# LukasHedegaard/continual-skeletons

Hardware: AMD Instinct MI355X
Metric: clips/sec (ST-GCN clip forward, NTU-60 shape; CoST-GCN online step reported under costgcn_online) (higher is better)
Workload: dtype f32

## Files before the change

### continual-skeletons_amd/blocks.py

```python
import math

import numpy as np
import torch
import torch.nn as nn
from torch.nn.modules.batchnorm import _BatchNorm
from torch.nn.modules.conv import _ConvNd

from . import fold, native


def init_weights(module_, bs=1):
    if isinstance(module_, _ConvNd):
        nn.init.constant_(module_.bias, 0)
        if bs == 1:
            nn.init.kaiming_normal_(module_.weight, mode="fan_out")
        else:
            nn.init.normal_(module_.weight, 0, math.sqrt(2.0 / (module_.weight.numel() * bs)))
    elif isinstance(module_, _BatchNorm):
        nn.init.constant_(module_.weight, bs)
        nn.init.constant_(module_.bias, 0)
    elif isinstance(module_, nn.Linear):
        nn.init.normal_(module_.weight, 0, math.sqrt(2.0 / bs))


def zero(x):
    return 0


def unity(x):
    return x


class _Folded(nn.Module):

    def _watched(self):
        return [self]

    def _snapshot(self):
        tensors, modules, seen = [], [(self._modules, tuple(self._modules.items()))], set()
        for root in self._watched():
            for m in root.modules():
                if id(m) in seen:
                    continue
                seen.add(id(m))
                for d in (m._parameters, m._buffers):
                    for name, t in d.items():
                        tensors.append((d, name, t, None if t is None else t.data_ptr(), None if t is None else t._version))
                modules.append((m._modules, tuple(m._modules.items())))
        return tensors, modules

    @staticmethod
    def _stale(snapshot):
        tensors, modules = snapshot
        for d, name, t, ptr, ver in tensors:
            cur = d.get(name)
            if cur is not t or (t is not None and (cur._version != ver or cur.data_ptr() != ptr)):
                return True
        for d, items in modules:
            if len(d) != len(items):
                return True
            for name, child in items:
                if d.get(name) is not child:
                    return True
        return False

    def _fingerprint(self):
        ts = [t for root in self._watched() for t in list(root.parameters()) + list(root.buffers())]
        return tuple((t.data_ptr(), t._version) for t in ts)

    def _packed_ops(self, device):
        cache = self.__dict__.get("_fold_cache")
        device = str(device)
        if cache is None or cache[0] != device or self._stale(cache[2]):
            ops = {k: (v.to(device) if isinstance(v, torch.Tensor) and not k.endswith("_host") else v)
                   for k, v in self._fold().items()}
            self.__dict__["_fold_cache"] = cache = (device, ops, self._snapshot())
        return cache[1]

    def refold(self):
        self.__dict__.pop("_fold_cache", None)

    def _require_eval(self):
        if self.training:
            raise RuntimeError(
                f"{type(self).__name__}: the MI355X path is inference-only (BatchNorm folded with running "
                "statistics); call .eval() first"
            )


PRECISIONS = ("f32", "bf16x3")


def set_precision(module: nn.Module, precision: str = "f32") -> nn.Module:
    if precision not in PRECISIONS:
        raise ValueError(f"precision must be one of {PRECISIONS}, got {precision!r}")
    blocks_ = [m for m in module.modules() if isinstance(m, SpatioTemporalBlock)]
    if not blocks_:
        raise ValueError("no SpatioTemporalBlock below this module: nothing to set")
    for m in blocks_:
        if precision != "f32" and not (m._native_tail and m.tcn.kernel_size == 9):
            raise NotImplementedError("bf16x3 is built for blocks with the native 9 x 1 temporal conv; the model is unchanged")
    for m in module.modules():
        if isinstance(m, SpatioTemporalBlock) or type(m) is GraphConvolution:
            m.precision = precision
            m.refold()
    return module


class SplitScratch:

    def __init__(self):
        self._bufs = {}

    def get(self, device, floats: int) -> torch.Tensor:
        key = (str(device), torch.cuda.current_stream(device).cuda_stream)
        bufs = self._bufs.setdefault(key, [])
        if not bufs or bufs[-1].numel() < floats:
            bufs.append(torch.empty(int(floats), device=device, dtype=torch.float32))
        return bufs[-1]

    def release(self):
        self._bufs.clear()

    def nbytes(self) -> int:
        return 4 * sum(b.numel() for bufs in self._bufs.values() for b in bufs)


def _scratch_of(module) -> SplitScratch:
    sc = module.__dict__.get("_split_scratch")
    if sc is None:
        sc = module.__dict__["_split_scratch"] = SplitScratch()
    return sc


CLIP_SPLIT_MAX_SEQUENCES = 6


def set_clip_latency_mode(module: nn.Module, split_k: int = 4, gcn_split_k: int = None, max_sequences: int = CLIP_SPLIT_MAX_SEQUENCES) -> nn.Module:
    gcn_split_k = split_k if gcn_split_k is None else gcn_split_k
    for v in (split_k, gcn_split_k):
        if not isinstance(v, int) or v < 0 or v > 32:
            raise ValueError("split_k must be an integer in [0, 32]")
    targets = [m for m in module.modules() if isinstance(m, SpatioTemporalBlock) or type(m) is GraphConvolution]
    if not targets:
        raise ValueError("no SpatioTemporalBlock / GraphConvolution below this module: nothing to set")
    if not isinstance(max_sequences, int) or max_sequences < 1:
        raise ValueError("max_sequences must be a positive integer")
    old = {id(sc): sc for sc in (m.__dict__.get("_split_scratch") for m in targets) if sc is not None}
    for sc in old.values():
        sc.release()
    shared = SplitScratch() if max(split_k, gcn_split_k) > 1 else None
    for m in targets:
        m.clip_split_k = split_k if isinstance(m, SpatioTemporalBlock) else gcn_split_k
        m.clip_split_max_seq = int(max_sequences)
        m.__dict__["_split_scratch"] = shared
    return module


def _check_input(x, channels, name):
    native.require_device_f32(x, name)
    if x.dim() != 4 or x.shape[1] != channels:
        raise RuntimeError(f"{name} must be (N, {channels}, T, V), got {tuple(x.shape)}")


class GraphConvolution(_Folded):

    def __init__(self, in_channels, out_channels, A, bn_momentum=0.1, *args, **kwargs):
        super().__init__()
        self.in_channels = in_channels
        self.out_channels = out_channels
        self.graph_attn = nn.Parameter(torch.ones(A.shape, dtype=torch.float32))
        self.A = nn.Parameter(torch.from_numpy(np.asarray(A).astype(np.float32)), requires_grad=False)
        self.num_subset = 3
        self.g_conv = nn.ModuleList(nn.Conv2d(in_channels, out_channels, 1) for _ in range(self.num_subset))
        for conv in self.g_conv:
            init_weights(conv, bs=self.num_subset)
        if in_channels != out_channels:
            self.gcn_residual = nn.Sequential(
                nn.Conv2d(in_channels, out_channels, 1), nn.BatchNorm2d(out_channels, momentum=bn_momentum)
            )
            init_weights(self.gcn_residual[0], bs=1)
            init_weights(self.gcn_residual[1], bs=1)
        else:
            self.gcn_residual = unity
        self.bn = nn.BatchNorm2d(out_channels, momentum=bn_momentum)
        init_weights(self.bn, bs=1e-6)
        self.relu = nn.ReLU()

    precision = "f32"

    def _fold(self):
        return fold.fold_graph_conv(self.state_dict(), split=self.precision == "bf16x3")

    def _split_applies(self, ops):
        cnt = ops["ell_cnt_host"]
        return (self.precision == "bf16x3" and ops["w_split"] is not None and self.out_channels % 128 == 0
                and int(cnt[0]) <= 1 and int(cnt[1]) <= 1 and int(cnt[2]) <= 4)

    def forward(self, x):
        self._require_eval()
        _check_input(x, self.in_channels, "GraphConvolution input")
        ops = self._packed_ops(x.device)
        n, c, t, v = x.shape
        if v != ops["V"]:
            raise RuntimeError(f"input has V={v} joints, adjacency has {ops['V']}")
        y = torch.empty((n, self.out_channels, t, v), device=x.device, dtype=torch.float32)
        if self._split_applies(ops):
            rc = native.lib().csk_gcn_stage_bf16x3(
                native.ptr(x), native.ptr(y), native.ptr(ops["w_split"]), native.ptr(ops["w_res_split"]), native.ptr(ops["bias"]),
                native.ptr(ops["ell_src"]), native.ptr(ops["ell_val"]), native.ptr(ops["ell_cnt_host"]), ops["ell_w"], n, c,
                self.out_channels, t, v, ops["res_mode"], native.stream_of(x))
            native.check(rc, "csk_gcn_stage_bf16x3")
            return y
        ks = self._clip_ksplit() if n <= self.clip_split_max_seq else 1
        if ks > 1:
            self.stage(x, y, n_seg=n, frames=t, x_strides=(c * t * v, t * v), y_strides=(self.out_channels * t * v, t * v),
                       ksplit=ks, partial=_scratch_of(self).get(x.device, ks * n * self.out_channels * t * v))
            return y
        gcn_stage(x, y, ops, n_seg=n, frames=t, x_strides=(c * t * v, t * v), y_strides=(self.out_channels * t * v, t * v))
        return y

    clip_split_k = 0
    clip_split_max_seq = CLIP_SPLIT_MAX_SEQUENCES

    def _clip_ksplit(self) -> int:
        if self.clip_split_k <= 1 or type(self) is not GraphConvolution or self.in_channels < 16:
            return 1
        return max(1, min(self.clip_split_k, -(-self.in_channels // 8)))

    def stage(self, x, y, n_seg, frames, x_strides, y_strides, ksplit=1, partial=None):
        ops = self._packed_ops(x.device)
        if ksplit > 1:
            rc = native.lib().csk_gcn_stage_splitk_f32(
                native.ptr(x), native.ptr(y), native.ptr(ops["w"]), native.ptr(ops["bias"]), native.ptr(ops["ell_src"]),
                native.ptr(ops["ell_val"]), native.ptr(ops["ell_cnt_host"]), ops["ell_w"], n_seg, ops["c_in"], ops["c_out"], frames,
                ops["V"], x_strides[0], x_strides[1], y_strides[0], y_strides[1], ops["res_mode"], ksplit, native.ptr(partial),
                native.stream_of(x))
            native.check(rc, "csk_gcn_stage_splitk_f32")
            return
        gcn_stage(x, y, ops, n_seg=n_seg, frames=frames, x_strides=x_strides, y_strides=y_strides)


def gcn_stage(x, y, ops, n_seg, frames, x_strides, y_strides, adj_seg_stride=0, adj_per_frame=0):
    rc = native.lib().csk_gcn_stage_f32(
        native.ptr(x), native.ptr(y), native.ptr(ops["w"]), native.ptr(ops["bias"]),
        native.ptr(ops["ell_src"]), native.ptr(ops["ell_val"]), native.ptr(ops["ell_cnt_host"]),
        ops["ell_w"], adj_seg_stride, adj_per_frame, n_seg, ops["c_in"], ops["c_out"], frames, ops["V"],
        x_strides[0], x_strides[1], y_strides[0], y_strides[1], ops["res_mode"], native.stream_of(x),
    )
    native.check(rc, "csk_gcn_stage_f32")


class TemporalConvolution(_Folded):

    def __init__(self, in_channels, out_channels, kernel_size=9, stride=1, padding=4):
        super().__init__()
        self.padding = padding
        self.stride = stride
        self.kernel_size = kernel_size
        self.t_conv = nn.Conv2d(in_channels, out_channels, kernel_size=(kernel_size, 1), padding=(padding, 0),
                                stride=(stride, 1))
        self.bn = nn.BatchNorm2d(out_channels)
        init_weights(self.t_conv, bs=1)
        init_weights(self.bn, bs=1)

    def _fold(self):
        f = fold.fold_temporal_conv(self.state_dict())
        f["bias"] = fold.pad_vec(f["bias"])
        return f

    def forward(self, x):
        self._require_eval()
        _check_input(x, self.t_conv.in_channels, "TemporalConvolution input")
        ops = self._packed_ops(x.device)
        return tcn_stage(x, ops["w"], ops["bias"], ops["c_out"], ops["k"], self.stride, self.padding, relu=False)


def tcn_stage(y, w, bias, c_out, k, stride, pad, relu=True, res_mode=0, x_res=None, w_res=None, res_off=0, out=None,
              split=False, ksplit=1, scratch=None):
    n, c, t_in, v = y.shape
    if t_in + 2 * pad < k:
        raise RuntimeError(f"temporal extent {t_in} (+2*{pad}) shorter than kernel {k}")
    t_out = (t_in + 2 * pad - k) // stride + 1
    if out is None:
        out = torch.empty((n, c_out, t_out, v), device=y.device, dtype=torch.float32)
    elif tuple(out.shape) != (n, c_out, t_out, v) or not out.is_contiguous() or out.dtype != torch.float32 or out.device != y.device:
        raise RuntimeError(f"out must be a contiguous float32 {(n, c_out, t_out, v)} tensor on {y.device}")
    c_res, t_res = (x_res.shape[1], x_res.shape[2]) if x_res is not None else (0, 0)
    if ksplit > 1 and not split:
        if scratch is None:
            raise RuntimeError("tcn_stage: ksplit > 1 needs the owning module's SplitScratch")
        part = scratch.get(y.device, ksplit * n * c_out * t_out * v)
        rc = native.lib().csk_tcn_stage_splitk_f32(
            native.ptr(y), native.ptr(w), native.ptr(x_res), native.ptr(w_res), native.ptr(bias), native.ptr(out),
            n, c, c_out, t_in, v, k, stride, pad, res_mode, c_res, t_res, res_off, int(relu), ksplit, native.ptr(part),
            native.stream_of(y))
        native.check(rc, "csk_tcn_stage_splitk_f32")
        return out
    fn = native.lib().csk_tcn_stage_bf16x3 if split else native.lib().csk_tcn_stage_f32
    rc = fn(native.ptr(y), native.ptr(w), native.ptr(x_res), native.ptr(w_res), native.ptr(bias), native.ptr(out),
            n, c, c_out, t_in, v, k, stride, pad, res_mode, c_res, t_res, res_off, int(relu), native.stream_of(y))
    native.check(rc, "csk_tcn_stage_bf16x3" if split else "csk_tcn_stage_f32")
    return out


class SpatioTemporalBlock(_Folded):

    def __init__(self, in_channels, out_channels, A, stride=1, residual=True, temporal_kernel_size=9,
                 temporal_padding=-1, GraphConv=GraphConvolution, TempConv=TemporalConvolution):
        super().__init__()
        equal_padding = int((temporal_kernel_size - 1) / 2)
        if temporal_padding < 0:
            temporal_padding = equal_padding
            self.residual_shrink = None
        else:
            assert temporal_padding <= equal_padding
            self.residual_shrink = equal_padding - temporal_padding
        self.stride = stride
        self.gcn = GraphConv(in_channels, out_channels, A)
        self.tcn = TempConv(out_channels, out_channels, stride=stride, kernel_size=temporal_kernel_size,
                            padding=temporal_padding)
        self.relu = nn.ReLU()
        if not residual:
            self.residual = zero
        elif (in_channels == out_channels) and (stride == 1):
            self.residual = unity
        else:
            self.residual = TempConv(in_channels, out_channels, kernel_size=1, stride=stride, padding=0)
        self._native_tail = isinstance(self.tcn, TemporalConvolution) and (
            self.residual in (zero, unity) or isinstance(self.residual, TemporalConvolution)
        )

    precision = "f32"
    clip_split_k = 0
    clip_split_max_seq = CLIP_SPLIT_MAX_SEQUENCES

    def _watched(self):
        return [m for m in (self.tcn, self.residual) if isinstance(m, nn.Module)]

    def _fold(self):
        sd = self.state_dict()
        return fold.fold_block_tail(sd, "", has_conv_residual=isinstance(self.residual, TemporalConvolution),
                                    split=self.precision == "bf16x3", stride=self.stride)

    def forward(self, x, out=None):
        self._require_eval()
        native.require_device_f32(x, "SpatioTemporalBlock input")
        if self._few_channels_fusable(x):
            return self._forward_few_channels(x, out)
        y = self.gcn(x)
        if not self._native_tail:
            z = self.tcn(y)
            r = self.residual(x[:, :, self.residual_shrink:-self.residual_shrink] if self.residual_shrink else x)
            return self.relu(z + r)
        ops = self._packed_ops(x.device)
        shrink = self.residual_shrink or 0
        if self.residual is zero:
            mode, xr = 0, None
        elif self.residual is unity:
            mode, xr = 1, x
        else:
            mode, xr = 2, x
        if self.precision == "bf16x3":
            return tcn_stage(y, ops["w_split"], ops["bias"], ops["c_out"], ops["k"], self.stride, self.tcn.padding, relu=True,
                             res_mode=mode, x_res=xr, w_res=ops["w_res_split"], res_off=shrink, out=out, split=True)
        ks = max(1, min(self.clip_split_k, -(-ops["c"] // 8))) if (self.clip_split_k > 1 and ops["k"] == 9 and y.shape[0] <= self.clip_split_max_seq) else 1
        return tcn_stage(y, ops["w"], ops["bias"], ops["c_out"], ops["k"], self.stride, self.tcn.padding, relu=True,
                         res_mode=mode, x_res=xr, w_res=ops["w_res"], res_off=shrink, out=out, ksplit=ks,
                         scratch=_scratch_of(self) if ks > 1 else None)


def _few_channels_fusable(self, x) -> bool:
    if not self.fuse_few_channels or type(self.gcn) is not GraphConvolution or not self._native_tail:
        return False
    if self.gcn.in_channels > 4 or self.residual is not zero or self.stride != 1 or self.precision != "f32" or self.residual_shrink:
        return False
    if x.dim() != 4 or x.shape[3] not in (18, 25) or self.gcn.precision != "f32":
        return False
    if self.clip_split_k > 1 and x.shape[0] <= self.clip_split_max_seq:
        return False
    g, t = self.gcn._packed_ops(x.device), self._packed_ops(x.device)
    return (t["k"] == 9 and self.tcn.padding == 4 and g["res_mode"] == 2 and g["c_out"] % 8 == 0 and g["V"] == x.shape[3]
            and max(int(v) for v in g["ell_cnt_host"][:2]) <= 1 and int(g["ell_cnt_host"][2]) <= 4)


def _forward_few_channels(self, x, out=None):
    _check_input(x, self.gcn.in_channels, "SpatioTemporalBlock input")
    g, t = self.gcn._packed_ops(x.device), self._packed_ops(x.device)
    n, c, tt, v = x.shape
    if out is None:
        out = torch.empty((n, t["c_out"], tt, v), device=x.device, dtype=torch.float32)
    rc = native.lib().csk_block_few_channels_f32(
        native.ptr(x.contiguous()), native.ptr(g["w"]), native.ptr(g["bias"]), native.ptr(g["ell_src"]), native.ptr(g["ell_val"]),
        native.ptr(g["ell_cnt_host"]), g["ell_w"], native.ptr(t["w"]), native.ptr(t["bias"]), native.ptr(out), n, c, g["c_out"],
        t["c_out"], tt, v, self.tcn.padding, native.stream_of(x))
    native.check(rc, "csk_block_few_channels_f32")
    return out


SpatioTemporalBlock.fuse_few_channels = False
SpatioTemporalBlock._few_channels_fusable = _few_channels_fusable
SpatioTemporalBlock._forward_few_channels = _forward_few_channels


def tcn_step_launch(*args):
    native.check(native.lib().csk_tcn_step_f32(*args), "csk_tcn_step_f32")
```

### continual-skeletons_amd/fold.py

```python
from typing import Dict, Optional, Tuple

import numpy as np
import torch

KC = 16
MT = 64
BN_EPS = 1e-5


def _ceil_to(a: int, b: int) -> int:
    return (a + b - 1) // b * b


def bn_affine(weight, bias, mean, var, eps=BN_EPS) -> Tuple[torch.Tensor, torch.Tensor]:
    s = weight.double() / torch.sqrt(var.double() + eps)
    return s, bias.double() - mean.double() * s


def pack_conv_weight(weight: torch.Tensor, scale: torch.Tensor) -> torch.Tensor:
    co, ci, k, _ = weight.shape
    w = weight.double()[:, :, :, 0] * scale[:, None, None]
    out = torch.zeros((k, _ceil_to(ci, KC), _ceil_to(co, MT)), dtype=torch.float64)
    out[:, :ci, :co] = w.permute(2, 1, 0)
    return out.float().contiguous()


SPLIT_KS = 16


def split3_bf16(w32: torch.Tensor):
    h = w32.to(torch.bfloat16)
    r1 = w32 - h.float()
    m = r1.to(torch.bfloat16)
    l = (r1 - m.float()).to(torch.bfloat16)
    return h, m, l


def pack_conv_weight_split(weight: torch.Tensor, scale: torch.Tensor, stride: int = 1) -> torch.Tensor:
    if weight.dim() == 4:
        weight = weight[:, :, :, 0]
    co, ci, k = weight.shape
    if k not in (1, 3, 9):
        raise ValueError(f"split weights are built for the 9 x 1 temporal conv, the 1 x 1 residual convs and the 3 graph-conv "
                         f"subsets, got k = {k}")
    w32 = (weight.double() * scale[:, None, None]).float()
    cpad, mpad = _ceil_to(ci, SPLIT_KS), _ceil_to(co, MT)
    taps = [r for rho in range(min(stride, k)) for r in range(rho, k, stride)] if k > 1 else [0]
    slots = _ceil_to(len(taps), 3)
    full = torch.zeros((mpad, cpad, slots), dtype=torch.float32)
    full[:co, :ci, : len(taps)] = w32[:, :, taps]
    pieces = torch.stack([p.view(torch.int16) for p in split3_bf16(full)], 0)
    out = pieces.view(3, mpad, cpad // SPLIT_KS, 2, 8, slots).permute(2, 5, 0, 3, 1, 4)
    return out.contiguous().reshape(-1)


def pad_vec(v: torch.Tensor) -> torch.Tensor:
    out = torch.zeros(_ceil_to(v.numel(), MT), dtype=torch.float64)
    out[: v.numel()] = v
    return out.float().contiguous()


def ell_from_dense(a_eff: torch.Tensor):
    a = a_eff.detach().cpu().double().numpy()
    three, v, _ = a.shape
    nz = a != 0
    per_col = nz.sum(axis=1)
    cnt = per_col.max(axis=1).astype(np.int32)
    ew = max(1, int(cnt.max()))
    src = np.zeros((three, v, ew), dtype=np.int32)
    val = np.zeros((three, v, ew), dtype=np.float32)
    for i in range(three):
        for w in range(v):
            rows = np.nonzero(nz[i, :, w])[0]
            src[i, w, : len(rows)] = rows
            val[i, w, : len(rows)] = a[i, rows, w]
    return torch.from_numpy(src), torch.from_numpy(val), torch.from_numpy(cnt), ew


def fold_graph_conv(sd: Dict[str, torch.Tensor], p: str = "", split: bool = False) -> dict:
    sd = {k: v.detach().cpu() for k, v in sd.items() if k.startswith(p)}
    s, t = bn_affine(sd[p + "bn.weight"], sd[p + "bn.bias"], sd[p + "bn.running_mean"], sd[p + "bn.running_var"])
    co, ci = sd[p + "g_conv.0.weight"].shape[:2]
    conv_res = (p + "gcn_residual.0.weight") in sd
    r = 4 if conv_res else 3
    w = torch.zeros((r, _ceil_to(ci, KC), _ceil_to(co, MT)), dtype=torch.float64)
    bias = t.clone()
    for i in range(3):
        w[i, :ci, :co] = (sd[f"{p}g_conv.{i}.weight"].double()[:, :, 0, 0] * s[:, None]).t()
        bias += s * sd[f"{p}g_conv.{i}.bias"].double()
    if conv_res:
        sr, tr = bn_affine(sd[p + "gcn_residual.1.weight"], sd[p + "gcn_residual.1.bias"],
                           sd[p + "gcn_residual.1.running_mean"], sd[p + "gcn_residual.1.running_var"])
        w[3, :ci, :co] = (sd[p + "gcn_residual.0.weight"].double()[:, :, 0, 0] * sr[:, None]).t()
        bias += sr * sd[p + "gcn_residual.0.bias"].double() + tr
    a_eff = sd[p + "A"].double() * sd[p + "graph_attn"].double()
    src, val, cnt, ew = ell_from_dense(a_eff)
    out = dict(w=w.float().contiguous(), bias=pad_vec(bias), ell_src=src, ell_val=val, ell_cnt_host=cnt,
               ell_w=ew, c_in=ci, c_out=co, res_mode=2 if conv_res else 1, V=a_eff.shape[-1], w_split=None, w_res_split=None)
    if split:
        one = torch.ones(co, dtype=torch.float64)
        w3 = w[:3, :ci, :co].permute(2, 1, 0).contiguous()
        out["w_split"] = pack_conv_weight_split(w3, one)
        if conv_res:
            out["w_res_split"] = pack_conv_weight_split(w[3, :ci, :co].t().contiguous().unsqueeze(-1), one)
    return out


def fold_temporal_conv(sd: Dict[str, torch.Tensor], p: str = "") -> dict:
    s, t = bn_affine(sd[p + "bn.weight"].cpu(), sd[p + "bn.bias"].cpu(), sd[p + "bn.running_mean"].cpu(),
                     sd[p + "bn.running_var"].cpu())
    wt = sd[p + "t_conv.weight"].detach().cpu()
    bias = s * sd[p + "t_conv.bias"].detach().cpu().double() + t
    return dict(w=pack_conv_weight(wt, s), bias=bias, c_in=wt.shape[1], c_out=wt.shape[0], k=wt.shape[2])


def fold_temporal_conv_split(sd: Dict[str, torch.Tensor], p: str = "", stride: int = 1) -> torch.Tensor:
    s, _ = bn_affine(sd[p + "bn.weight"].cpu(), sd[p + "bn.bias"].cpu(), sd[p + "bn.running_mean"].cpu(),
                     sd[p + "bn.running_var"].cpu())
    return pack_conv_weight_split(sd[p + "t_conv.weight"].detach().cpu(), s, stride)


def fold_block_tail(sd: Dict[str, torch.Tensor], p: str = "", has_conv_residual: Optional[bool] = None,
                    split: bool = False, stride: int = 1) -> dict:
    main = fold_temporal_conv(sd, p + "tcn.")
    out = dict(w=main["w"], k=main["k"], c=main["c_in"], c_out=main["c_out"], w_res=None, c_res=0, w_split=None, w_res_split=None)
    bias = main["bias"]
    if has_conv_residual is None:
        has_conv_residual = (p + "residual.t_conv.weight") in sd
    if has_conv_residual:
        res = fold_temporal_conv(sd, p + "residual.")
        out["w_res"], out["c_res"] = res["w"], res["c_in"]
        bias = bias + res["bias"]
    if split:
        out["w_split"] = fold_temporal_conv_split(sd, p + "tcn.", stride)
        if has_conv_residual:
            out["w_res_split"] = fold_temporal_conv_split(sd, p + "residual.")
    out["bias"] = pad_vec(bias)
    return out


def fold_data_bn(sd: Dict[str, torch.Tensor], p: str = "data_bn."):
    s, t = bn_affine(sd[p + "weight"].cpu(), sd[p + "bias"].cpu(), sd[p + "running_mean"].cpu(),
                     sd[p + "running_var"].cpu())
    return s.float().contiguous(), t.float().contiguous()
```

### continual-skeletons_amd/native.py

```python
import ctypes as C
import os

import torch

_HERE = os.path.dirname(os.path.abspath(__file__))
LIB_PATH = os.path.join(_HERE, "libcskel_hip.so")
ABI_VERSION = 15

_p, _i, _l = C.c_void_p, C.c_int, C.c_int64
SIGNATURES = {
    "csk_abi_version": [],
    "csk_stream_overlap_probe": [C.c_void_p, C.c_void_p, C.c_int, C.POINTER(C.c_float)],
    "csk_gcn_stage_f32": [_p, _p, _p, _p, _p, _p, _p, _i, _l, _i, _i, _i, _i, _i, _i, _l, _l, _l, _l, _i, _p],
    "csk_gcn_stage_splitk_f32": [_p, _p, _p, _p, _p, _p, _p, _i, _i, _i, _i, _i, _i, _l, _l, _l, _l, _i, _i, _p, _p],
    "csk_tcn_stage_f32": [_p, _p, _p, _p, _p, _p, _i, _i, _i, _i, _i, _i, _i, _i, _i, _i, _i, _i, _i, _p],
    "csk_block_few_channels_f32": [_p, _p, _p, _p, _p, _p, _i, _p, _p, _p, _i, _i, _i, _i, _i, _i, _i, _p],
    "csk_tcn_stage_splitk_f32": [_p, _p, _p, _p, _p, _p, _i, _i, _i, _i, _i, _i, _i, _i, _i, _i, _i, _i, _i, _i, _p, _p],
    "csk_conv1x1_f32": [_p, _p, _p, _p, _i, _i, _i, _i, _i, _l, _l, _l, _l, _p],
    "csk_tcn_stage_bf16x3": [_p, _p, _p, _p, _p, _p, _i, _i, _i, _i, _i, _i, _i, _i, _i, _i, _i, _i, _i, _p],
    "csk_gcn_stage_bf16x3": [_p, _p, _p, _p, _p, _p, _p, _p, _i, _i, _i, _i, _i, _i, _i, _p],
    "csk_input_norm_f32": [_p, _p, _p, _p, _i, _i, _i, _i, _i, _l, _l, _p],
    "csk_pool_fc_f32": [_p, _p, _p, _p, _p, _i, _i, _i, _i, _i, _p],
    "csk_fc_f32": [_p, _p, _p, _p, _i, _i, _i, _p],
    "csk_pool_scaled_f32": [_p, _p, _i, _i, _i, _i, C.c_float, _p],
    "csk_agcn_attention_f32": [_p, _p, _p, _p, _i, _i, _i, _i, _l, _l, _i, _l, _p],
    "csk_agcn_embed_attention_f32": [_p, _p, _p, _p, _p, _p, _i, _i, _i, _i, _i, _i, _l, _l, _p],
    "csk_tcn_step_f32": [_p, _i, _i, _i, _i, _p, _p, _i, _i, _i, _p, _p, _p, _i, _i, _i, _i, _l, _i, _i, _i, _i, _i, _p, _p],
    "csk_co_stack_step_f32": [_i, _p, _i, _i, _l, _p],
    "csk_co_block_step_f32": [_p, _i, _i, _i, _p, _p, _p, _p, _p, _i, _i, _p, _i, _i, _p, _p, _i, _i, _p, _i, _i, _i, _i, _i, _l, _p],
    "csk_co_spatial_pool_f32": [_p, _p, _i, _i, _i, _l, _p],
    "csk_co_window_mean_f32": [_p, _p, _l, _i, _i, _i, _p],
    "csk_co_head_step_f32": [_p, _p, _p, _p, _p, _p, _i, _i, _i, _l, _i, _i, _i, _i, _i, _p],
    "csk_input_norm_frames_f32": [_p, _p, _i, _p, _p, _i, _i, _i, _i, _l, _p],

    "csk_fuse_rank_f32": [_p, _i, _i, _i, _i, _l, _l, _p, _p, _p, _p],
    "csk_co_plan_create": [_i, _p, _p, _i, _i, _i, _i, _i, _l, _p, _p, _i, _p, _p, _i, _i, _p, _p],
    "csk_co_plan_destroy": [_p],
    "csk_co_plan_update_weights": [_p, _i, _p, _p, _p, _p, _p],
    "csk_co_plan_reset": [_p],
    "csk_co_plan_counters": [_p, C.POINTER(C.c_int64), _i, _i],
    "csk_co_plan_set_fusion": [_p, _i],
    "csk_co_plan_cycle": [_p, _p, _i, _p, _p, _p, _p, _p],
}
RESTYPES = {"csk_co_plan_create": C.c_void_p, "csk_co_plan_destroy": None, "csk_co_plan_reset": None}


class CoLayer(C.Structure):
    _fields_ = [("c_in", C.c_int32), ("c_out", C.c_int32), ("stride", C.c_int32), ("res_kind", C.c_int32),
                ("gcn_res_mode", C.c_int32), ("ell_w", C.c_int32), ("ell_cnt", C.c_int32 * 3), ("tcn_ksplit", C.c_int32),
                ("y_slots", C.c_int32), ("out_slots", C.c_int32), ("partial_emits", C.c_int32), ("agcn_adj_frames", C.c_int32),
                ("gcn_ksplit", C.c_int32), ("gcn_partial_frames", C.c_int32),
                ("gcn_w", C.c_void_p), ("gcn_bias", C.c_void_p), ("ell_src", C.c_void_p), ("ell_val", C.c_void_p),
                ("tcn_w", C.c_void_p), ("tcn_w_res", C.c_void_p), ("tcn_bias", C.c_void_p),
                ("y_ring", C.c_void_p), ("out_ring", C.c_void_p), ("tcn_partial", C.c_void_p),
                ("agcn_inter", C.c_int32), ("agcn_pad_", C.c_int32), ("agcn_w_pairs", C.c_void_p), ("agcn_b_pairs", C.c_void_p),
                ("agcn_a_sum", C.c_void_p), ("agcn_adj", C.c_void_p)]


_lib = None


def lib():
    global _lib
    if _lib is None:
        if not os.path.exists(LIB_PATH):
            raise RuntimeError(
                f"{LIB_PATH} not found: the HIP library is not built. "
                "Run `python -c 'import __graft_entry__ as g; g.build()'` (needs hipcc); there is no CPU fallback."
            )
        handle = C.CDLL(LIB_PATH)
        for name, args in SIGNATURES.items():
            fn = getattr(handle, name)
            fn.argtypes = args
            fn.restype = RESTYPES.get(name, C.c_int)
        handle.csk_last_error.restype = C.c_char_p
        handle.csk_last_error.argtypes = []
        if handle.csk_abi_version() != ABI_VERSION:
            raise RuntimeError("libcskel_hip.so ABI version mismatch; rebuild it")
        _lib = handle
    return _lib


def check(rc: int, what: str):
    if rc == 0:
        return
    if rc < 0:
        raise RuntimeError(f"{what}: {lib().csk_last_error().decode()}")
    raise RuntimeError(f"{what}: HIP launch failed with hipError_t {rc}")


def ptr(t):
    return None if t is None else C.c_void_p(t.data_ptr())


def stream_of(t: torch.Tensor):
    return C.c_void_p(torch.cuda.current_stream(t.device).cuda_stream)


def require_device_f32(t: torch.Tensor, name: str):
    if not isinstance(t, torch.Tensor):
        raise TypeError(f"{name} must be a torch.Tensor")
    if not t.is_cuda:
        raise RuntimeError(
            f"{name} is on {t.device}: this is the MI355X-native path and has no CPU fallback "
            "(move the module and its inputs to a ROCm device)"
        )
    if t.dtype != torch.float32:
        raise RuntimeError(f"{name} must be float32, got {t.dtype}")
    if not t.is_contiguous():
        raise RuntimeError(f"{name} must be contiguous")
```

### include/cskel.h

```cpp
#ifndef CSKEL_H
#define CSKEL_H

#include <stdint.h>

#ifdef __cplusplus
extern "C" {
#endif

#define CSK_ABI_VERSION 15
#define CSK_KC 8
#define CSK_CPAD 16
#define CSK_MT 64

#define CSK_RES_NONE 0
#define CSK_RES_IDENTITY 1
#define CSK_RES_CONV 2

int csk_abi_version(void);
const char *csk_last_error(void);

int csk_stream_overlap_probe(void *stream_a, void *stream_b, int spin_us, float *ratio);

int csk_gcn_stage_f32(const float *x, float *y, const float *w, const float *bias,
                      const int32_t *ell_src, const float *ell_val, const int32_t *ell_cnt,
                      int ell_w, int64_t adj_seg_stride, int adj_per_frame,
                      int n_seg, int c_in, int c_out, int frames, int V,
                      int64_t x_seg_stride, int64_t x_chan_stride,
                      int64_t y_seg_stride, int64_t y_chan_stride,
                      int res_mode, void *stream);

int csk_gcn_stage_splitk_f32(const float *x, float *y, const float *w, const float *bias, const int32_t *ell_src,
                             const float *ell_val, const int32_t *ell_cnt, int ell_w, int n_seg, int c_in, int c_out,
                             int frames, int V, int64_t x_seg_stride, int64_t x_chan_stride, int64_t y_seg_stride,
                             int64_t y_chan_stride, int res_mode, int ksplit, float *partial, void *stream);

int csk_tcn_stage_f32(const float *y, const float *w, const float *x_res, const float *w_res,
                      const float *bias, float *out,
                      int n_seg, int c, int c_out, int t_in, int V, int k, int stride, int pad,
                      int res_mode, int c_res, int t_res, int res_off, int relu, void *stream);

int csk_block_few_channels_f32(const float *x, const float *gcn_w, const float *gcn_bias, const int32_t *ell_src,
                               const float *ell_val, const int32_t *ell_cnt, int ell_w, const float *tcn_w,
                               const float *tcn_bias, float *out, int n_seg, int c_in, int c_mid, int c_out, int t_in,
                               int V, int pad, void *stream);

int csk_tcn_stage_splitk_f32(const float *y, const float *w, const float *x_res, const float *w_res,
                             const float *bias, float *out,
                             int n_seg, int c, int c_out, int t_in, int V, int k, int stride, int pad,
                             int res_mode, int c_res, int t_res, int res_off, int relu, int ksplit, float *partial,
                             void *stream);

int csk_conv1x1_f32(const float *x, float *y, const float *w, const float *bias, int n_seg, int c_in, int c_out,
                    int frames, int V, int64_t x_seg_stride, int64_t x_chan_stride, int64_t y_seg_stride,
                    int64_t y_chan_stride, void *stream);

int csk_tcn_stage_bf16x3(const float *y, const void *w_split, const float *x_res, const void *w_res_split,
                         const float *bias, float *out,
                         int n_seg, int c, int c_out, int t_in, int V, int k, int stride, int pad,
                         int res_mode, int c_res, int t_res, int res_off, int relu, void *stream);

int csk_gcn_stage_bf16x3(const float *x, float *y, const void *w_split, const void *w_res_split, const float *bias,
                         const int32_t *ell_src, const float *ell_val, const int32_t *ell_cnt, int ell_w,
                         int n_seg, int c_in, int c_out, int frames, int V, int res_mode, void *stream);

int csk_input_norm_f32(const float *x, const float *scale, const float *shift, float *h,
                       int N, int C, int T, int V, int M,
                       int64_t h_seg_stride, int64_t h_chan_stride, void *stream);

int csk_pool_fc_f32(const float *h, const float *fc_w, const float *fc_b, float *feat, float *logits,
                    int N, int M, int C, int TV, int classes, void *stream);

int csk_pool_scaled_f32(const float *h, float *feat, int N, int M, int C, int TV, float scale, void *stream);

int csk_fc_f32(const float *feat, const float *fc_w, const float *fc_b, float *logits,
               int N, int C, int classes, void *stream);

int csk_agcn_attention_f32(const float *E, const float *a_sum, float *ell_val, float *scratch, int n_seg, int inter, int T,
                           int V, int64_t e_seg_stride, int64_t e_chan_stride, int seg_per_group, int64_t e_group_stride,
                           void *stream);

int csk_agcn_embed_attention_f32(const float *x, const float *w_pairs, const float *b_pairs, const float *a_sum, float *ell_val,
                                 float *scratch, int n_seg, int c_in, int inter, int frames, int V, int per_frame,
                                 int64_t x_seg_stride, int64_t x_chan_stride, void *stream);


int csk_tcn_step_f32(const float *ring, int slots, int head, int head_step, int n_emit, const float *w,
                     const float *x_res, int x_res_slots, int x_res_slot0, int x_res_step,
                     const float *w_res, const float *bias, float *out, int out_slots, int out_slot0,
                     int c, int c_out, int64_t P, int k, int res_mode, int c_res, int relu, int ksplit, float *partial,
                     void *stream);

int csk_co_block_step_f32(const float *xin, int xin_slots, int xin_slot0, int c_in, const float *gcn_w,
                          const float *gcn_bias, const int32_t *ell_src, const float *ell_val, const int32_t *ell_cnt,
                          int ell_w, int gcn_res_mode, float *y_ring, int y_slots, int y_slot0, const float *tcn_w,
                          const float *tcn_bias, int res_mode, int x_res_slot0, float *out, int out_slots, int out_slot0,
                          int c_out, int n_skel, int V, int64_t P, void *stream);

#define CSK_CO_STACK_MAX 4
typedef struct csk_co_block_args {
    const float *xin;
    int32_t xin_slots, xin_slot0, c_in;
    const float *gcn_w, *gcn_bias;
    const int32_t *ell_src;
    const float *ell_val;
    int32_t ell_cnt[3], ell_w, gcn_res_mode;
    float *y_ring;
    int32_t y_slots, y_slot0;
    const float *tcn_w, *tcn_bias;
    int32_t res_mode, x_res_slot0;
    float *out;
    int32_t out_slots, out_slot0, c_out;
} csk_co_block_args;
int csk_co_stack_step_f32(int n_blocks, const csk_co_block_args *blocks, int n_skel, int V, int64_t P, void *stream);

int csk_co_spatial_pool_f32(const float *h, float *feat, int N, int C, int MV, int64_t P, void *stream);

int csk_co_window_mean_f32(const float *ring, float *pooled, int64_t n_elem, int window, int head, int count,
                           void *stream);

int csk_co_head_step_f32(const float *h, float *pool_ring, float *pooled, const float *fc_w, const float *fc_b, float *logits,
                         int N, int C, int MV, int64_t P, int window, int head, int count, int emit, int classes, void *stream);

int csk_input_norm_frames_f32(const float *const *frames, float *const *dst, int r, const float *scale, const float *shift,
                              int N, int C, int V, int M, int64_t P, void *stream);

int csk_fuse_rank_f32(const float *const *preds, int n_streams, int use_max, int N, int classes,
                      int64_t sample_stride, int64_t class_stride, const int64_t *targets, float *fused, int *rank,
                      void *stream);

#define CSK_CO_MAX_CYCLE 8
#define CSK_CO_Y_SLOTS(max_in) (8 + (max_in))
#define CSK_CO_IN_SLOTS(max_in) (4 + (max_in))

typedef struct csk_co_layer {
    int32_t c_in, c_out, stride, res_kind;
    int32_t gcn_res_mode, ell_w, ell_cnt[3];
    int32_t tcn_ksplit;
    int32_t y_slots, out_slots;
    int32_t partial_emits;
    int32_t agcn_adj_frames;
    int32_t gcn_ksplit, gcn_partial_frames;
    const float *gcn_w, *gcn_bias;
    const int32_t *ell_src;
    const float *ell_val;
    const float *tcn_w, *tcn_w_res, *tcn_bias;
    float *y_ring;
    float *out_ring;
    float *tcn_partial;
    int32_t agcn_inter, agcn_pad_;
    const float *agcn_w_pairs, *agcn_b_pairs, *agcn_a_sum;
    float *agcn_adj;
} csk_co_layer;

typedef struct csk_co_plan csk_co_plan;

csk_co_plan *csk_co_plan_create(int n_layers, const csk_co_layer *layers, float *xin0, int xin0_slots, int N, int C, int V, int M,
                                int64_t P, const float *bn_scale, const float *bn_shift, int classes,
                                const float *fc_w, const float *fc_b, int pool_size, int pool_padding,
                                float *pool_ring, float *pooled);
void csk_co_plan_destroy(csk_co_plan *plan);
int csk_co_plan_update_weights(csk_co_plan *plan, int n_layers, const csk_co_layer *layers, const float *bn_scale,
                               const float *bn_shift, const float *fc_w, const float *fc_b);
void csk_co_plan_reset(csk_co_plan *plan);
int csk_co_plan_counters(csk_co_plan *plan, int64_t *buf, int n, int set);
int csk_co_plan_set_fusion(csk_co_plan *plan, int enable);
int csk_co_plan_cycle(csk_co_plan *plan, const float *const *frames, int r, float *logits, int *last_slot,
                      int *n_feat, int *n_logits, void *stream);

#ifdef __cplusplus
}
#endif
#endif
```

Baseline: 3673.

## Add Winograd F(2,3)-based temporal conv kernel for stride-1 identity-residual blocks

Adds a HIP kernel that computes the 9-tap temporal convolution as three F(2,3) Winograd groups. Weights are pre-transformed at fold time into a 12-tap image, and inputs are transformed on the fly inside the MFMA inner loop. It produces two output frames per column and cuts multiply work from 9 to 12/2 per output. The new path runs only for k=9, stride 1, identity residual and V of 18 or 25, and falls back to the existing kernel otherwise. It adds small numerical differences from the Winograd transform and puts extra ALU work in the inner loop.

```diff
diff --git a/continual-skeletons_amd/blocks.py b/continual-skeletons_amd/blocks.py
--- a/continual-skeletons_amd/blocks.py
+++ b/continual-skeletons_amd/blocks.py
@@ -277,7 +277,7 @@
 
 
 def tcn_stage(y, w, bias, c_out, k, stride, pad, relu=True, res_mode=0, x_res=None, w_res=None, res_off=0, out=None,
-              split=False, ksplit=1, scratch=None):
+              split=False, ksplit=1, scratch=None, w_wino=None):
     n, c, t_in, v = y.shape
     if t_in + 2 * pad < k:
         raise RuntimeError(f"temporal extent {t_in} (+2*{pad}) shorter than kernel {k}")
@@ -296,6 +296,13 @@
             n, c, c_out, t_in, v, k, stride, pad, res_mode, c_res, t_res, res_off, int(relu), ksplit, native.ptr(part),
             native.stream_of(y))
         native.check(rc, "csk_tcn_stage_splitk_f32")
+        return out
+    if w_wino is not None and not split:
+        rc = native.lib().csk_tcn_stage_wino_f32(
+            native.ptr(y), native.ptr(w), native.ptr(x_res), native.ptr(w_res), native.ptr(bias), native.ptr(out),
+            n, c, c_out, t_in, v, k, stride, pad, res_mode, c_res, t_res, res_off, int(relu), native.ptr(w_wino),
+            native.stream_of(y))
+        native.check(rc, "csk_tcn_stage_wino_f32")
         return out
     fn = native.lib().csk_tcn_stage_bf16x3 if split else native.lib().csk_tcn_stage_f32
     rc = fn(native.ptr(y), native.ptr(w), native.ptr(x_res), native.ptr(w_res), native.ptr(bias), native.ptr(out),
@@ -367,7 +374,7 @@
         ks = max(1, min(self.clip_split_k, -(-ops["c"] // 8))) if (self.clip_split_k > 1 and ops["k"] == 9 and y.shape[0] <= self.clip_split_max_seq) else 1
         return tcn_stage(y, ops["w"], ops["bias"], ops["c_out"], ops["k"], self.stride, self.tcn.padding, relu=True,
                          res_mode=mode, x_res=xr, w_res=ops["w_res"], res_off=shrink, out=out, ksplit=ks,
-                         scratch=_scratch_of(self) if ks > 1 else None)
+                         scratch=_scratch_of(self) if ks > 1 else None, w_wino=ops["w_wino"] if ks == 1 else None)
 
 
 def _few_channels_fusable(self, x) -> bool:
diff --git a/continual-skeletons_amd/csrc/tcn_wino.hip b/continual-skeletons_amd/csrc/tcn_wino.hip
--- /dev/null
+++ b/continual-skeletons_amd/csrc/tcn_wino.hip
@@ -0,0 +1,212 @@
+#include "mfma_core.h"
+#include "tcn_params.h"
+
+namespace {
+
+constexpr int WMT = 64;
+constexpr int WNT = 128;
+constexpr int WTAPS = 12;
+
+template <int VT>
+constexpr int wino_ldb() { return ((2 * ((WNT + VT - 2) / VT) + 10) * VT + 3) / 4 * 4; }
+
+struct WStage12x64 {
+    unsigned goff0, loff0, gstride;
+    f32x4 v[6];
+    __device__ __forceinline__ void setup(int Cpad, int Mpad, int tid) {
+        goff0 = (unsigned)(((tid >> 7) * Cpad + ((tid >> 4) & 7)) * Mpad + (tid & 15) * 4);
+        loff0 = (unsigned)(tid * 4);
+        gstride = (unsigned)(2 * Cpad * Mpad);
+    }
+    __device__ __forceinline__ void issue_slot(int u, const float *__restrict__ chunk_base) {
+        v[u] = *reinterpret_cast<const f32x4 *>(chunk_base + (size_t)u * gstride + goff0);
+    }
+    __device__ __forceinline__ void issue(const float *__restrict__ chunk_base) {
+#pragma unroll
+        for (int u = 0; u < 6; ++u) issue_slot(u, chunk_base);
+    }
+    __device__ __forceinline__ void commit(float *__restrict__ Wl) const {
+#pragma unroll
+        for (int u = 0; u < 6; ++u) *reinterpret_cast<f32x4 *>(Wl + u * (NTHREADS * 4) + loff0) = v[u];
+    }
+};
+
+template <int VT, int G>
+__device__ __forceinline__ void wino_group(const float *__restrict__ Wl, const float *__restrict__ Bl, int off, int l31, int kh,
+                                           f32x16 (&acc)[4][2]) {
+    constexpr int LDB = wino_ldb<VT>();
+    const float *br = Bl + kh * LDB + off + 3 * G * VT;
+    const float *wr = Wl + 4 * G * (KC * WMT) + kh * WMT + l31;
+#pragma unroll
+    for (int s = 0; s < KC / 2; ++s) {
+        const float d0 = br[2 * s * LDB], d1 = br[2 * s * LDB + VT], d2 = br[2 * s * LDB + 2 * VT], d3 = br[2 * s * LDB + 3 * VT];
+        const float b[4] = {d0 - d2, d1 + d2, d2 - d1, d1 - d3};
+#pragma unroll
+        for (int i = 0; i < 4; ++i) {
+            const float a0 = wr[i * (KC * WMT) + 2 * s * WMT], a1 = wr[i * (KC * WMT) + 2 * s * WMT + 32];
+            acc[i][0] = __builtin_amdgcn_mfma_f32_32x32x2f32(a0, b[i], acc[i][0], 0, 0, 0);
+            acc[i][1] = __builtin_amdgcn_mfma_f32_32x32x2f32(a1, b[i], acc[i][1], 0, 0, 0);
+        }
+    }
+}
+
+}
+
+template <int VT>
+__global__ __launch_bounds__(NTHREADS, 2) void tcn_stage_wino_kernel(const TcnParams p) {
+    constexpr int LDB = wino_ldb<VT>();
+    constexpr int NJ = (LDB + 63) / 64;
+    extern __shared__ __attribute__((aligned(16))) float smem[];
+    float *Wl = smem;
+    float *Bl = smem + WTAPS * KC * WMT;
+
+    const int tid = threadIdx.x, lane = tid & 63, wave = __builtin_amdgcn_readfirstlane(tid >> 6);
+    const int l31 = lane & 31, kh = lane >> 5;
+    const unsigned wid = xcd_contiguous_id(blockIdx.x, gridDim.x);
+    const int m0 = (int)(wid % p.mtiles) * WMT, q0 = (int)((wid / p.mtiles) % p.qtiles) * WNT;
+    const int seg = (int)(wid / (p.mtiles * p.qtiles));
+    const int T = p.Tout, TV = T * VT, QP = p.nt;
+    const int qend = min(q0 + WNT, QP);
+    const int ja = div_magic(q0, p.vmagic), jb = div_magic(qend - 1, p.vmagic);
+
+    const int qc = min(q0 + wave * 32 + l31, qend - 1);
+    const int jc = div_magic(qc, p.vmagic), vc = qc - jc * VT;
+    const int off = 2 * (jc - ja) * VT + vc;
+
+    f32x16 acc[4][2];
+#pragma unroll
+    for (int i = 0; i < 4; ++i)
+#pragma unroll
+        for (int mi = 0; mi < 2; ++mi)
+#pragma unroll
+            for (int g = 0; g < 16; ++g) acc[i][mi][g] = 0.f;
+
+    {
+        const int fa = 2 * ja - 4;
+        const int span = (2 * (jb - ja) + 10) * VT;
+        const int64_t cs = (int64_t)TV;
+        const float *seg_base = p.y + (int64_t)seg * p.C * cs;
+        const float *wbase = p.w + m0;
+        WStage12x64 ws;
+        ws.setup(p.Cpad, p.Mpad, tid);
+        auto kloop = [&](auto &bx) {
+            ws.issue(wbase);
+            bx.issue(seg_base, p.C, cs, 0, wave);
+            for (int c0 = 0; c0 + KC < p.Cpad; c0 += KC) {
+                __syncthreads();
+                ws.commit(Wl);
+                bx.commit(Bl, LDB, wave);
+                __syncthreads();
+                const float *wnext = wbase + (size_t)(c0 + KC) * p.Mpad;
+                const int cn = c0 + KC;
+                ws.issue_slot(0, wnext);
+                ws.issue_slot(1, wnext);
+                bx.template issue_third<0>(seg_base, p.C, cs, cn, wave);
+                if (p.prio) __builtin_amdgcn_s_setprio(1);
+                wino_group<VT, 0>(Wl, Bl, off, l31, kh, acc);
+                __builtin_amdgcn_s_setprio(0);
+                ws.issue_slot(2, wnext);
+                ws.issue_slot(3, wnext);
+                bx.template issue_third<1>(seg_base, p.C, cs, cn, wave);
+                if (p.prio) __builtin_amdgcn_s_setprio(1);
+                wino_group<VT, 1>(Wl, Bl, off, l31, kh, acc);
+                __builtin_amdgcn_s_setprio(0);
+                ws.issue_slot(4, wnext);
+                ws.issue_slot(5, wnext);
+                bx.template issue_third<2>(seg_base, p.C, cs, cn, wave);
+                if (p.prio) __builtin_amdgcn_s_setprio(1);
+                wino_group<VT, 2>(Wl, Bl, off, l31, kh, acc);
+                __builtin_amdgcn_s_setprio(0);
+            }
+            __syncthreads();
+            ws.commit(Wl);
+            bx.commit(Bl, LDB, wave);
+            __syncthreads();
+            wino_group<VT, 0>(Wl, Bl, off, l31, kh, acc);
+            wino_group<VT, 1>(Wl, Bl, off, l31, kh, acc);
+            wino_group<VT, 2>(Wl, Bl, off, l31, kh, acc);
+        };
+        const bool interior = p.vec_stage && fa >= 0 && fa * VT + 4 * ((span + 3) / 4) <= TV;
+        if (interior) {
+            BStage4<(NJ + 3) / 4> b4;
+            b4.setup(fa * VT, span, lane);
+            kloop(b4);
+        } else {
+            BStage<NJ> bs;
+            bs.setup(fa * VT, span, TV, lane);
+            kloop(bs);
+        }
+    }
+
+    const bool qv = q0 + wave * 32 + l31 < qend;
+    const bool odd_ok = 2 * jc + 1 < T;
+    const unsigned p0 = (unsigned)(2 * jc * VT + vc);
+    const unsigned b0 = 4u * (4u * (unsigned)kh * (unsigned)TV + p0);
+    const unsigned b1 = odd_ok ? b0 + 4u * VT : b0;
+    const unsigned kh16 = 16u * (unsigned)kh;
+    const float *rseg = p.xres + (int64_t)seg * p.Cout * TV;
+    float *oseg = p.out + (int64_t)seg * p.Cout * TV;
+#pragma unroll
+    for (int mi = 0; mi < 2; ++mi) {
+        const int rb = m0 + mi * 32;
+        float o0[16], o1[16];
+#pragma unroll
+        for (int g = 0; g < 16; ++g) {
+            const int row = rb + (g & 3) + 8 * (g >> 2);
+            const float *rrow = rseg + (int64_t)row * TV;
+            const float bias = ld_lane(p.bias + row, kh16);
+            const float m1 = acc[1][mi][g], m2 = acc[2][mi][g];
+            float v0 = acc[0][mi][g] + m1 + m2 + bias + ld_lane(rrow, b0);
+            float v1 = m1 - m2 - acc[3][mi][g] + bias + ld_lane(rrow, b1);
+            if (p.relu) { v0 = relu_nan(v0); v1 = relu_nan(v1); }
+            o0[g] = v0;
+            o1[g] = v1;
+        }
+        if (qv) {
+#pragma unroll
+            for (int g = 0; g < 16; ++g) {
+                float *orow = oseg + (int64_t)(rb + (g & 3) + 8 * (g >> 2)) * TV;
+                st_lane(orow, b0, o0[g]);
+                if (odd_ok) st_lane(orow, b1, o1[g]);
+            }
+        }
+    }
+}
+
+static int tcn_stage_wino_launch(const float *y, const float *w_wino, const float *x_res, const float *bias, float *out, int n_seg,
+                                 int c, int c_out, int t_in, int V, int k, int stride, int pad, int res_mode, int c_res, int t_res,
+                                 int res_off, int relu, void *stream) {
+    if (!w_wino || !y || !x_res || !bias || !out) return -2;
+    if (k != 9 || stride != 1 || pad != 4 || res_mode != CSK_RES_IDENTITY || res_off != 0) return -2;
+    if ((V != 25 && V != 18) || c_out % WMT != 0 || c_res != c_out || t_res != t_in || c < 1 || n_seg < 1 || t_in < 1) return -2;
+    if ((int64_t)t_in * V >= (1 << 26)) return -2;
+    if (csk_diag_flag("CSK_TCN_WINO")) return -2;
+    const int qp = (t_in + 1) / 2 * V;
+    const int qtiles = (qp + WNT - 1) / WNT, mtiles = c_out / WMT;
+    if ((int64_t)qtiles * mtiles * n_seg >= (1ll << 31)) return -2;
+    TcnParams p = {};
+    p.y = y; p.w = w_wino; p.xres = x_res; p.wres = nullptr; p.bias = bias; p.out = out;
+    p.C = c; p.Cpad = round_up(c, CSK_CPAD); p.Cout = c_out; p.Mpad = round_up(c_out, CSK_MT);
+    p.Tin = t_in; p.Tout = t_in; p.V = V; p.K = k; p.stride = 1; p.pad = pad;
+    p.res_mode = res_mode; p.Cres = c_res; p.CresPad = round_up(c_res, CSK_CPAD); p.Tres = t_res; p.res_off = 0; p.relu = relu;
+    p.vmagic = vmagic_of(V); p.mtiles = (unsigned)mtiles; p.qtiles = (unsigned)qtiles; p.nt = qp;
+    p.prio = !csk_diag_flag("CSK_NOPRIO");
+    p.vec_stage = !csk_diag_flag("CSK_TCN_NOVEC");
+    void (*kern)(TcnParams) = V == 25 ? tcn_stage_wino_kernel<25> : tcn_stage_wino_kernel<18>;
+    const int ldb = V == 25 ? wino_ldb<25>() : wino_ldb<18>();
+    p.ldb = ldb;
+    const size_t lds = (size_t)(WTAPS * KC * WMT + KC * ldb) * sizeof(float);
+    if (const int e = csk_ensure_lds((const void *)kern, lds)) return e;
+    hipLaunchKernelGGL(kern, dim3((unsigned)(qtiles * mtiles * n_seg)), dim3(NTHREADS), lds, (hipStream_t)stream, p);
+    return (int)hipGetLastError();
+}
+
+extern "C" int csk_tcn_stage_wino_f32(const float *y, const float *w, const float *x_res, const float *w_res, const float *bias,
+                                      float *out, int n_seg, int c, int c_out, int t_in, int V, int k, int stride, int pad,
+                                      int res_mode, int c_res, int t_res, int res_off, int relu, const float *w_wino, void *stream) {
+    const int rc = tcn_stage_wino_launch(y, w_wino, x_res, bias, out, n_seg, c, c_out, t_in, V, k, stride, pad, res_mode, c_res,
+                                         t_res, res_off, relu, stream);
+    if (rc != -2) return rc;
+    return csk_tcn_stage_f32(y, w, x_res, w_res, bias, out, n_seg, c, c_out, t_in, V, k, stride, pad, res_mode, c_res, t_res,
+                             res_off, relu, stream);
+}
diff --git a/continual-skeletons_amd/fold.py b/continual-skeletons_amd/fold.py
--- a/continual-skeletons_amd/fold.py
+++ b/continual-skeletons_amd/fold.py
@@ -22,6 +22,23 @@
     w = weight.double()[:, :, :, 0] * scale[:, None, None]
     out = torch.zeros((k, _ceil_to(ci, KC), _ceil_to(co, MT)), dtype=torch.float64)
     out[:, :ci, :co] = w.permute(2, 1, 0)
+    return out.float().contiguous()
+
+
+WINO_G = ((1.0, 0.0, 0.0), (0.5, 0.5, 0.5), (0.5, -0.5, 0.5), (0.0, 0.0, 1.0))
+
+
+def pack_conv_weight_wino(weight: torch.Tensor, scale: torch.Tensor) -> torch.Tensor:
+    if weight.dim() == 4:
+        weight = weight[:, :, :, 0]
+    co, ci, k = weight.shape
+    if k != 9:
+        raise ValueError(f"the Winograd image is built for the 9 x 1 temporal conv, got k = {k}")
+    w = weight.double() * scale[:, None, None]
+    g = torch.tensor(WINO_G, dtype=torch.float64)
+    u = torch.einsum("ir,ocgr->gico", g, w.view(co, ci, 3, 3)).reshape(12, ci, co)
+    out = torch.zeros((12, _ceil_to(ci, KC), _ceil_to(co, MT)), dtype=torch.float64)
+    out[:, :ci, :co] = u
     return out.float().contiguous()
 
 
@@ -106,12 +123,13 @@
     return out
 
 
-def fold_temporal_conv(sd: Dict[str, torch.Tensor], p: str = "") -> dict:
+def fold_temporal_conv(sd: Dict[str, torch.Tensor], p: str = "", wino: bool = False) -> dict:
     s, t = bn_affine(sd[p + "bn.weight"].cpu(), sd[p + "bn.bias"].cpu(), sd[p + "bn.running_mean"].cpu(),
                      sd[p + "bn.running_var"].cpu())
     wt = sd[p + "t_conv.weight"].detach().cpu()
     bias = s * sd[p + "t_conv.bias"].detach().cpu().double() + t
-    return dict(w=pack_conv_weight(wt, s), bias=bias, c_in=wt.shape[1], c_out=wt.shape[0], k=wt.shape[2])
+    w_wino = pack_conv_weight_wino(wt, s) if wino and wt.shape[2] == 9 else None
+    return dict(w=pack_conv_weight(wt, s), bias=bias, c_in=wt.shape[1], c_out=wt.shape[0], k=wt.shape[2], w_wino=w_wino)
 
 
 def fold_temporal_conv_split(sd: Dict[str, torch.Tensor], p: str = "", stride: int = 1) -> torch.Tensor:
@@ -122,8 +140,9 @@
 
 def fold_block_tail(sd: Dict[str, torch.Tensor], p: str = "", has_conv_residual: Optional[bool] = None,
                     split: bool = False, stride: int = 1) -> dict:
-    main = fold_temporal_conv(sd, p + "tcn.")
-    out = dict(w=main["w"], k=main["k"], c=main["c_in"], c_out=main["c_out"], w_res=None, c_res=0, w_split=None, w_res_split=None)
+    main = fold_temporal_conv(sd, p + "tcn.", wino=stride == 1)
+    out = dict(w=main["w"], k=main["k"], c=main["c_in"], c_out=main["c_out"], w_res=None, c_res=0, w_split=None, w_res_split=None,
+               w_wino=main["w_wino"])
     bias = main["bias"]
     if has_conv_residual is None:
         has_conv_residual = (p + "residual.t_conv.weight") in sd
diff --git a/continual-skeletons_amd/native.py b/continual-skeletons_amd/native.py
--- a/continual-skeletons_amd/native.py
+++ b/continual-skeletons_amd/native.py
@@ -14,6 +14,7 @@
     "csk_gcn_stage_f32": [_p, _p, _p, _p, _p, _p, _p, _i, _l, _i, _i, _i, _i, _i, _i, _l, _l, _l, _l, _i, _p],
     "csk_gcn_stage_splitk_f32": [_p, _p, _p, _p, _p, _p, _p, _i, _i, _i, _i, _i, _i, _l, _l, _l, _l, _i, _i, _p, _p],
     "csk_tcn_stage_f32": [_p, _p, _p, _p, _p, _p, _i, _i, _i, _i, _i, _i, _i, _i, _i, _i, _i, _i, _i, _p],
+    "csk_tcn_stage_wino_f32": [_p, _p, _p, _p, _p, _p, _i, _i, _i, _i, _i, _i, _i, _i, _i, _i, _i, _i, _i, _p, _p],
     "csk_block_few_channels_f32": [_p, _p, _p, _p, _p, _p, _i, _p, _p, _p, _i, _i, _i, _i, _i, _i, _i, _p],
     "csk_tcn_stage_splitk_f32": [_p, _p, _p, _p, _p, _p, _i, _i, _i, _i, _i, _i, _i, _i, _i, _i, _i, _i, _i, _i, _p, _p],
     "csk_conv1x1_f32": [_p, _p, _p, _p, _i, _i, _i, _i, _i, _l, _l, _l, _l, _p],
diff --git a/include/cskel.h b/include/cskel.h
--- a/include/cskel.h
+++ b/include/cskel.h
@@ -38,6 +38,11 @@
                       const float *bias, float *out,
                       int n_seg, int c, int c_out, int t_in, int V, int k, int stride, int pad,
                       int res_mode, int c_res, int t_res, int res_off, int relu, void *stream);
+
+int csk_tcn_stage_wino_f32(const float *y, const float *w, const float *x_res, const float *w_res,
+                           const float *bias, float *out,
+                           int n_seg, int c, int c_out, int t_in, int V, int k, int stride, int pad,
+                           int res_mode, int c_res, int t_res, int res_off, int relu, const float *w_wino, void *stream);
 
 int csk_block_few_channels_f32(const float *x, const float *gcn_w, const float *gcn_bias, const int32_t *ell_src,
                                const float *ell_val, const int32_t *ell_cnt, int ell_w, const float *tcn_w,
```

Result: faster. 4076, median of 6 (+11.0%).
